# RunhuiWang/DeltaPQ

Measured on AMD Instinct MI355X. Metric: queries/sec, SIFT1M-shaped m=8 k=256 topk=100, higher is better.
Workload: dtype f64 sum of f32 table entries (u8 code decode; the reference's incremental f64 stack); 1 GPU

## Files before the change

deltapq_amd/_lib.py:

```python
import ctypes
import os

_HERE = os.path.dirname(os.path.abspath(__file__))
LIB_PATH = os.environ.get("DPQ_LIB_PATH") or os.path.join(_HERE, "csrc", "libdeltapq_amd.so")

c_i32, c_i64, c_f32 = ctypes.c_int32, ctypes.c_int64, ctypes.c_float
P = ctypes.POINTER


class OpenOpts(ctypes.Structure):
    _fields_ = [("device", c_i32), ("shard_rank", c_i32), ("shard_count", c_i32), ("chunks_per_segment", c_i32),
                ("cand_capacity", c_i32), ("num_codes", c_i32), ("bootstrap", c_i32), ("batch_decode", c_i32),
                ("global_offset", c_i64), ("global_n_codes", c_i64),
                ("stream_max_queries", c_i32), ("coarse_below", c_i32), ("plan_ratios", c_i32 * 3), ("boot_cap", c_i32),
                ("boot_target", c_i32), ("flags", c_i32), ("batch_tile_nodes", c_i64)]


class Info(ctypes.Structure):
    _fields_ = [("n_codes_total", c_i64), ("n_bytes_total", c_i64), ("node_lo", c_i64), ("node_hi", c_i64),
                ("algorithmic_bytes", c_i64), ("device_bytes", c_i64), ("n_diffs", c_i64), ("M", c_i32),
                ("K", c_i32), ("Ds", c_i32), ("n_segments", c_i32), ("chunks_per_segment", c_i32),
                ("max_depth", c_i32), ("device", c_i32), ("cand_capacity", c_i32), ("bootstrap_bytes", c_i64),
                ("bootstrap_stride", c_i32), ("batch_decode_mb", c_i32), ("strand_bytes", c_i64)]

# ... 205 lines not shown
    ("dpq_ip_tables", ctypes.c_int, [_VP, _VP, ctypes.c_int, _VP, _VP]),
    ("dpq_ip_tables_device", ctypes.c_int, [_VP, _VP, ctypes.c_int, _VP, _VP, _VP]),
    ("dpq_query_batch_ip", ctypes.c_int, [_VP, _VP, _VP, ctypes.c_int, ctypes.c_int, _VP, _VP, _VP, _VP]),
    ("dpq_query_batch_device_ip", ctypes.c_int, [_VP, _VP, _VP, ctypes.c_int, ctypes.c_int, _VP, _VP, _VP, _VP, _VP]),
    ("dpq_ip_scores", ctypes.c_int, [_VP, _VP, _VP, ctypes.c_int, ctypes.c_int, _VP]),
    ("dpq_profile_enable", ctypes.c_int, [_VP, ctypes.c_int]),
    ("dpq_profile_reset", ctypes.c_int, [_VP]),
    ("dpq_profile_read", ctypes.c_int, [_VP, P(Profile)]),
    ("dpq_debug_scan_time", ctypes.c_int, [_VP, ctypes.c_int, ctypes.c_int, ctypes.c_int, ctypes.c_int, P(ctypes.c_float)]),
    ("dpq_debug_scan_stamps", ctypes.c_int, [_VP, ctypes.c_int, ctypes.c_int, P(ctypes.c_ulonglong), ctypes.c_int, P(ctypes.c_float)]),
    ("dpq_debug_boot_stamps", ctypes.c_int, [_VP, ctypes.c_int, P(ctypes.c_double)]),
    ("dpq_debug_select_time", ctypes.c_int, [_VP, ctypes.c_int, ctypes.c_int, ctypes.c_int, ctypes.c_int, P(ctypes.c_float)]),
    ("dpq_debug_strand1_stamps", ctypes.c_int, [_VP, _VP, ctypes.c_int]),
    ("dpq_debug_range_keys", ctypes.c_int, [_VP, P(c_i64)]),
    ("dpq_debug_filter_tables", ctypes.c_int, [_VP, ctypes.c_int, _VP, c_i64]),
    ("dpq_debug_relabel", ctypes.c_int, [_VP, _VP, ctypes.c_int]),
]

_lib = None
_hip_runtime = None


def _bind_hip_runtime():
    global _hip_runtime
    if _hip_runtime is not None:
        return _hip_runtime
    import importlib.util
    candidates = []
    override = os.environ.get("DPQ_HIP_RUNTIME")
    if override:
# ... 52 lines not shown
```

deltapq_amd/api.py:

```python
import ctypes

import numpy as np

from . import _lib
from ._lib import DpqError, Info, OpenOpts, Profile, check


def _np_ptr(a):
    return ctypes.c_void_p(a.ctypes.data)


def device_count():
    return _lib.load().dpq_device_count()


def read_codewords(path):
    lib = _lib.load()
    M, K, Ds = _lib.c_i32(), _lib.c_i32(), _lib.c_i32()
    check(lib.dpq_read_codewords(path.encode(), M, K, Ds, None), "dpq_read_codewords")
    out = np.empty((M.value, K.value, Ds.value), dtype=np.float32)
    check(lib.dpq_read_codewords(path.encode(), M, K, Ds, _np_ptr(out)), "dpq_read_codewords")
    return out


# ... 392 lines not shown
    def info(self):
        i = Info()
        check(self._lib.dpq_get_info(self._h, i), "dpq_get_info")
        return i.as_dict()

    def query_batch(self, queries, top_k):
        q = np.ascontiguousarray(queries, dtype=np.float32)
        if q.ndim == 1:
            q = q[None, :]
        nq = q.shape[0]
        ids = np.empty((nq, top_k), dtype=np.int32)
        dists = np.empty((nq, top_k), dtype=np.float32)
        check(self._lib.dpq_query_batch(self._h, _np_ptr(q), nq, top_k, _np_ptr(ids), _np_ptr(dists)),
              "dpq_query_batch")
        return ids, dists

    def range_search(self, queries, radius):
        q = np.ascontiguousarray(queries, dtype=np.float32)
        if q.ndim == 1:
            q = q[None, :]
        nq = q.shape[0]
        r = np.ascontiguousarray(np.broadcast_to(np.asarray(radius, dtype=np.float32), (nq,)))
        res = ctypes.c_void_p()
        check(self._lib.dpq_range_search(self._h, _np_ptr(q), nq, _np_ptr(r), res), "dpq_range_search")
        try:
            n = _lib.c_i32()
            pl, pi, pd = ctypes.c_void_p(), ctypes.c_void_p(), ctypes.c_void_p()
            check(self._lib.dpq_range_result_get(res, n, pl, pi, pd), "dpq_range_result_get")
            lims = np.ctypeslib.as_array(ctypes.cast(pl, ctypes.POINTER(_lib.c_i64)), (n.value + 1,)).copy()
            total = int(lims[-1])
# ... 1119 lines not shown
```

deltapq_amd/csrc/dpq_capi.cpp:

```cpp
#include "dpq_capi_internal.h"

namespace {

thread_local std::string g_last_error;

}

int fail(int code, const std::string& msg) {
    g_last_error = msg;
    return code;
}

uint64_t next_index_serial() {
    static std::atomic<uint64_t> next{1};
    return next++;
}

bool dev_mode() {
    const char* dev = getenv("DPQ_DEV");
    return dev && atoi(dev) != 0;
}

namespace {

// ... 22 lines not shown
        geti("DPQ_BOOT_TARGET", &t.boot_target);
        geti("DPQ_BOOT_VARIANT", &t.boot_variant);
        if (const char* e = getenv("DPQ_BATCH_TILE_NODES")) t.batch_tile_nodes = std::max<int64_t>(1, atoll(e));
        int v = 1;
        geti("DPQ_RELABEL", &v); t.relabel = t.relabel && v != 0;
        v = 1; geti("DPQ_FUSE_QUANTISE", &v); t.fuse_quantise = t.fuse_quantise && v != 0;
        v = 1; geti("DPQ_ASYNC_OVERLAP", &v); t.async_overlap = t.async_overlap && v != 0;
        v = 0; geti("DPQ_BOOT_FULLSORT", &v); t.boot_fullsort = t.boot_fullsort || v != 0;
        v = 1; geti("DPQ_TIGHTEN", &v); t.tighten = t.tighten && v != 0;
        geti("DPQ_SELECT_THREADS", &t.select_threads);
        geti("DPQ_SELECT_FAST", &t.select_fast);
        v = 1; geti("DPQ_STRANDS", &v); t.strands = t.strands && v != 0;
        t.force_strands = t.force_strands || v == 2;
        v = 1; geti("DPQ_STRAND1", &v); t.strand1 = t.strand1 && v != 0;
        geti("DPQ_S1_DEBUG", &t.s1_debug);
    }
    return t;
}

void use_lane(dpq_index* x, int lane) {
    if (lane == x->active_lane) return;
    x->dbg_groups = x->dbg_boot_slots = 0;
    x->active_lane = lane;
}

int ensure_workspace(dpq_index* x, int slots, int cap) {
    Workspace& w = x->ws();
    if (slots <= w.slots && cap <= w.cap) return DPQ_OK;
    slots = std::max(slots, w.slots);
    cap = std::max(cap, w.cap);
    x->dbg_groups = x->dbg_boot_slots = 0;
    DevBuf<uint8_t> batch_raw = std::move(w.d_batch_raw);
    w = Workspace();
    w.d_batch_raw = std::move(batch_raw);
    int rc;
    if ((rc = w.d_lut32.alloc((size_t)slots * x->M * 256))) return rc;
    if (x->d_relabel && (rc = w.d_lut32r.alloc((size_t)slots * x->M * 256))) return rc;
    if ((rc = w.d_lut_min.alloc((size_t)slots * x->M * 4))) return rc;
    if ((rc = w.d_lut_stat.alloc((size_t)slots * x->M))) return rc;
    if ((rc = w.d_qtab.alloc((size_t)(slots / dpq::queries_per_group(x->M) + 1) *
                             (dpq::qtab_bytes_per_group(x->M) / sizeof(uint4)))))
        return rc;
    if ((rc = w.d_cand_count.alloc((size_t)slots * dpq::kRegionStride))) return rc;
    if ((rc = w.d_cand_key.alloc((size_t)slots * cap))) return rc;
    if ((rc = w.d_scratch.alloc((size_t)slots * cap))) return rc;
    if ((rc = w.d_overflow.alloc((size_t)slots))) return rc;
    if ((rc = w.d_tight.alloc((size_t)slots * dpq::kTightWords))) return rc;
    if ((rc = w.d_thr_key.alloc((size_t)slots))) return rc;
    if ((rc = w.d_dbg_thr.alloc((size_t)slots))) return rc;
    if (!x->h_overflow) DPQ_HIP(hipHostMalloc(reinterpret_cast<void**>(&x->h_overflow), sizeof(uint32_t) * 4096));
    if (!x->d_counters) {
        if ((rc = x->d_counters.alloc(2))) return rc;
        DPQ_HIP(hipMemset(x->d_counters, 0, 16));
    }
// ... 248 lines not shown
    if (stride > INT32_MAX) return fail(DPQ_ERR_NOMEM, "candidate buffer too large");
    if ((rc = ensure_workspace(x, b->nqp, (int)stride))) return rc;
    b->stride = x->ws().cap;
    if (b->scratch && (rc = ensure_batch_raw(x))) return rc;
    return DPQ_OK;
}

int build_tables(dpq_index* x, const Batch& b, const TableSource& src, hipStream_t stream, bool row_stats = true) {
    Workspace& w = x->ws();
    int rc;
    if (b.one_tile && (rc = ensure_plain_image(x, stream))) return rc;
    {
        Timer t(x, stream, 0);
        const uint8_t* relabel = b.scratch ? x->d_relabel.get() : nullptr;
        uint32_t* tight = x->tune.tighten ? w.d_tight.get() : nullptr;
        if (src.d_tables)
            DPQ_HIP(dpq::launch_tables_ingest(src.d_tables, b.nq, b.nqp, x->M, x->K, w.d_lut32, w.d_lut_min, w.d_overflow,
                                              relabel, w.d_lut32r, tight, src.d_bad, stream));
        else
            DPQ_HIP(dpq::launch_lut_build(x->d_codebook, src.d_queries, b.nq, b.nqp, x->M, x->K, x->Ds, w.d_lut32,
                                          w.d_lut_min, nullptr, w.d_overflow, relabel, w.d_lut32r, tight, stream));
        if (row_stats) DPQ_HIP(dpq::launch_row_stats(w.d_lut32, b.nq, x->M, w.d_lut_stat, stream));
    }
    if (x->prof) x->prof_acc.lut_launches++;
    return DPQ_OK;
}

dpq::ScanArgs batch_scan_args(const dpq_index* x, const Batch& b) {
    const Workspace& w = x->ws();
    dpq::ScanArgs sa{};
    sa.img = x->img;
    if (b.one_tile) sa.img.raw = x->d_plain_image;
    sa.fp32_accum = x->plain ? 1 : 0;
    sa.lut32 = b.labelled ? w.d_lut32r.get() : w.d_lut32.get();
    sa.lut_min = w.d_lut_min;
    sa.lut_stat = w.d_lut_stat;
    sa.thr_key = w.d_thr_key;
// ... 1731 lines not shown
        int rc;
        if ((rc = d_rec.alloc(records))) return rc;
        dpq::ScanArgs sa{};
        sa.img.M = x->M;
        sa.lut_min = w.d_lut_min;
        sa.lut_stat = w.d_lut_stat;
        sa.thr_key = w.d_dbg_thr;
        sa.n_queries = w.dbg_qtab_nq;
        DPQ_HIP(dpq::launch_saturation_debug(sa, slots, d_rec, nullptr));
        DPQ_HIP(hipMemcpy(static_cast<char*>(out) + tables, d_rec.get(), records, hipMemcpyDeviceToHost));
    }
    return DPQ_OK;
    });
}

int dpq_debug_relabel(dpq_index* x, unsigned char* out, int bytes) {
    return guarded([&]() -> int {
    DPQ_DEV_ONLY();
    if (!x || !out || bytes < x->M * 256) return fail(DPQ_ERR_ARG, "bad argument");
    if (!x->d_relabel) return fail(DPQ_ERR_STATE, "the handle has no label map");
    DPQ_HIP(hipSetDevice(x->device));
    DPQ_HIP(hipDeviceSynchronize());
    DPQ_HIP(hipMemcpy(out, x->d_relabel.get(), (size_t)x->M * 256, hipMemcpyDeviceToHost));
    return DPQ_OK;
    });
}

int dpq_debug_range_keys(dpq_index* x, int64_t* max_keys) {
    DPQ_DEV_ONLY();
    if (!x || !max_keys) return fail(DPQ_ERR_ARG, "NULL argument");
// ... 102 lines not shown
```

deltapq_amd/csrc/dpq_capi_internal.h:

```cpp
#pragma once
#include <hip/hip_runtime.h>

#include <algorithm>
#include <atomic>
#include <chrono>
#include <cmath>
#include <cstdio>
#include <cstdlib>
#include <cstring>
#include <iterator>
#include <memory>
#include <new>
#include <numeric>
#include <stdexcept>
#include <string>
#include <type_traits>
#include <vector>

#include "../../include/deltapq_amd.h"
#include "dpq_build.h"
#include "dpq_filter.h"
#include "dpq_flat.h"
#include "dpq_format.h"
#include "dpq_kernels.h"
// ... 145 lines not shown
uint64_t next_index_serial();

struct Tuning {
    int stream_max = 4;
    int coarse_below = 128;
    int plan_ratios[3] = {0, 0, 0};
    int boot_cap = 0, boot_target = 0;
    int boot_variant = 1;
    int select_threads = 0;
    int select_fast = 1;
    int64_t batch_tile_nodes = (int64_t)16 << 20;
    bool relabel = true, fuse_quantise = true, async_overlap = true, boot_fullsort = false, tighten = true, strands = true,
         force_strands = false;
    bool strand1 = true;
    int s1_debug = 0;
};

struct RangeWs {
    DevBuf<int32_t> slot_query;
    DevBuf<uint64_t> thr_key;
    DevBuf<int64_t> out_off;
    DevBuf<uint32_t> max_count;
    DevBuf<int64_t> lims;
    DevBuf<uint32_t> cand_count;
    DevBuf<uint64_t> cand_key;
    DevBuf<int32_t> out_ids;
    DevBuf<float> out_dists;
    DevBuf<uint64_t> scratch;
    size_t key_n = 0, out_n = 0, scratch_n = 0;
    int64_t last_max_keys = 0;
// ... 10 lines not shown
};

struct TableSource {
    const float* d_queries = nullptr;
    const float* d_tables = nullptr;
    uint32_t* d_bad = nullptr;
    const float* h_tables = nullptr;
};

struct Workspace {
    int slots = 0, cap = 0;
    DevBuf<float> d_lut32;
    DevBuf<float> d_lut32r;
    DevBuf<float> d_lut_min;
    DevBuf<float> d_lut_stat;
    DevBuf<uint4> d_qtab;
    DevBuf<uint32_t> d_cand_count;
    DevBuf<uint32_t> d_overflow;
    DevBuf<uint32_t> d_tight;
    DevBuf<uint64_t> d_cand_key, d_thr_key;
    DevBuf<uint64_t> d_scratch;
    DevBuf<uint8_t> d_batch_raw;
    int dbg_qtab_groups = 0, dbg_qtab_levels = 0;
    int dbg_qtab_nq = 0;
    DevBuf<uint64_t> d_dbg_thr;
};

struct dpq_index {
    Tuning tune;
    const uint64_t serial = next_index_serial();
// ... 144 lines not shown
```

deltapq_amd/csrc/dpq_kernels.h:

```cpp
#pragma once
#include <hip/hip_runtime.h>

#include <cstdint>

#include "dpq_format.h"

namespace dpq {

constexpr int kScanThreads = 1024;
constexpr int kScanWaves = kScanThreads / 64;
constexpr int kMaxTopK = 2048;
constexpr int kSelectThreads = 512;
constexpr int kMaxSplits = 256;
constexpr int kRegionStride = 1 + kMaxSplits;
constexpr int kLevel0Nodes = 3840;
constexpr int kSortMax = 4096;
constexpr int queries_per_group(int M) { return M <= 8 ? 64 : 32; }
constexpr int kTightBuckets = 8;
constexpr int kTightSplits = 32;
constexpr int kTightWords = kTightSplits * kTightBuckets / 4;
constexpr int kS1Replicas = 8, kS1ReplicaWords = 512;
constexpr int kS1HistWords = kS1Replicas * kS1ReplicaWords;
static_assert(queries_per_group(8) * kTightWords >= kS1HistWords, "strand1's histogram exceeds what one query group clears");
constexpr int kLutQueries = 8;
constexpr int kLutMinParts = 4;

struct DeviceImage {
    const uint8_t* nib = nullptr;
    const uint8_t* par = nullptr;
    const uint8_t* carry = nullptr;
    const uint8_t* mask = nullptr;
    const uint8_t* delta = nullptr;
    const uint64_t* seg_delta_off = nullptr;
    const uint8_t* seg_ckpt = nullptr;
    const uint8_t* raw = nullptr;
    const uint64_t* st_ckpt = nullptr;
    const uint32_t* st_mask = nullptr;
    const uint16_t* st_depth = nullptr;
    const uint32_t* st_pbase = nullptr;
    const uint8_t* st_delta = nullptr;
// ... 106 lines not shown
    const int64_t* out_off;
    const uint32_t* cand_count;
    const uint64_t* cand_key;
    int64_t cand_stride;
    int32_t region_off, region_cap, n_regions;
    int32_t lds_keys;
    int32_t* out_ids;
    float* out_dists;
    int64_t out_n;
    uint64_t* scratch;
    int64_t n_codes_total;
};

hipError_t launch_lut_build(const float* d_codebook, const float* d_queries, int nq, int n_slots, int M, int K, int Ds,
                            float* d_lut32, float* d_lut_min, uint32_t* d_cand_count, uint32_t* d_overflow,
                            const uint8_t* d_relabel, float* d_lut_labels, uint32_t* d_tight_hist,
                            hipStream_t stream);
hipError_t launch_decode_list(const DeviceImage& img, const uint32_t* seg_list, int n_seg, const uint8_t* relabel,
                              uint32_t* out_code, hipStream_t stream);
hipError_t launch_decode_segments(const DeviceImage& img, const uint32_t* seg_list, int n_seg, uint32_t* out_id,
                                  uint32_t* out_code, hipStream_t stream);
hipError_t launch_stream(const ScanArgs& a, int n_slots, hipStream_t stream);
hipError_t launch_strand(const ScanArgs& a, int n_slots, hipStream_t stream);
int stream_queries_per_pass(int M, int n_slots);
hipError_t launch_strand1(const ScanArgs& a, int n_slots, hipStream_t stream);
int strand1_workgroups(int n_strips);
constexpr int kStrand1Regions = 256;
hipError_t launch_quantise(const ScanArgs& a, int n_slot_groups, hipStream_t stream);
hipError_t launch_row_stats(const float* d_lut32, int nq, int M, float* d_lut_stat, hipStream_t stream);
hipError_t launch_scan(const ScanArgs& a, int n_slot_groups, int splits, hipStream_t stream);
size_t qtab_bytes_per_group(int M);
hipError_t launch_saturation_debug(const ScanArgs& a, int n_slots, unsigned char* d_out, hipStream_t stream);
// ... 14 lines not shown
```

deltapq_amd/csrc/dpq_kernels.hip:

```cpp
#include "dpq_kernels.h"
#include "dpq_wave_decoder.h"

#include <atomic>
#include <type_traits>
#include <cfloat>
#include <cmath>

namespace dpq {

static hipError_t ensure_dynamic_lds(const void* fn, size_t bytes, std::atomic<bool>* done);


__device__ __forceinline__ uint32_t and_or(uint32_t a, uint32_t mask, uint32_t c) {
    uint32_t r;
    asm("v_and_or_b32 %0, %1, %2, %3" : "=v"(r) : "v"(a), "s"(mask), "v"(c));
    return r;
}

__device__ __forceinline__ uint64_t make_key(float d, uint32_t id) {
    return ((uint64_t)__float_as_uint(d) << 32) | (uint64_t)id;
}

__device__ __forceinline__ float lut_min_of(const float* __restrict__ lut_min, size_t q, int M, int m) {
    const float4 p = *reinterpret_cast<const float4*>(lut_min + (q * M + m) * kLutMinParts);
    return fminf(fminf(p.x, p.y), fminf(p.z, p.w));
}

__global__ __launch_bounds__(256) void lut_build_kernel(const float* __restrict__ codebook,
                                                         const float* __restrict__ queries, int nq, int n_slots, int M,
                                                         int K, int Ds, float* __restrict__ lut,
                                                         float* __restrict__ lut_min, uint32_t* __restrict__ cand_count,
                                                         uint32_t* __restrict__ overflow, const uint8_t* __restrict__ relabel,
                                                         float* __restrict__ lut_labels, uint32_t* __restrict__ tight_hist) {
#ifndef DPQ_UNDER_SCAN_PRIO
#define DPQ_UNDER_SCAN_PRIO 3
#endif
    __builtin_amdgcn_s_setprio(DPQ_UNDER_SCAN_PRIO);
    const int q0 = blockIdx.x * kLutQueries, m = blockIdx.y, k = threadIdx.x;
    if (m == 0 && k < kLutQueries && q0 + k < n_slots) {
        if (cand_count) cand_count[q0 + k] = 0;
        if (overflow) overflow[q0 + k] = 0;
    }
    if (m == 0 && tight_hist)
        for (int i = k; i < kLutQueries * kTightWords; i += 256)
            if (q0 * kTightWords + i < n_slots * kTightWords) tight_hist[(size_t)q0 * kTightWords + i] = 0;
    if (q0 >= nq) return;
    float acc[kLutQueries];
#pragma unroll
    for (int j = 0; j < kLutQueries; ++j) acc[j] = 0.0f;
    if (k < K) {
        const float* c = codebook + ((size_t)m * K + k) * Ds;
        const float* qv = queries + (size_t)q0 * M * Ds + (size_t)m * Ds;
        const size_t qstride = (size_t)M * Ds;
        auto step = [&](float& a, float cv, float qd) {
            const float diff = __fsub_rn(cv, qd);
            const double sq = __dmul_rn((double)diff, (double)diff);
            a = (float)__dadd_rn((double)a, sq);
        };
        if ((Ds & 3) == 0) {
            const float4* c4 = reinterpret_cast<const float4*>(c);
            for (int d = 0; d < Ds; d += 4) {
                const float4 v = c4[d >> 2];
#pragma unroll
                for (int j = 0; j < kLutQueries; ++j) {
                    const float* qj = qv + (size_t)min(j, nq - 1 - q0) * qstride + d;
                    step(acc[j], v.x, qj[0]);
                    step(acc[j], v.y, qj[1]);
                    step(acc[j], v.z, qj[2]);
                    step(acc[j], v.w, qj[3]);
                }
            }
        } else {
            for (int d = 0; d < Ds; ++d) {
                const float cv = c[d];
#pragma unroll
                for (int j = 0; j < kLutQueries; ++j) step(acc[j], cv, qv[(size_t)min(j, nq - 1 - q0) * qstride + d]);
            }
        }
    } else {
#pragma unroll
        for (int j = 0; j < kLutQueries; ++j) acc[j] = INFINITY;
    }
#pragma unroll
    for (int j = 0; j < kLutQueries; ++j) {
        if (q0 + j < nq) lut[((size_t)(q0 + j) * M + m) * 256 + k] = acc[j];
        if (lut_labels && q0 + j < nq) lut_labels[((size_t)(q0 + j) * M + m) * 256 + relabel[m * 256 + k]] = acc[j];
        uint32_t v = __float_as_uint(acc[j]);
#pragma unroll
        for (int o = 32; o > 0; o >>= 1) v = min(v, (uint32_t)__shfl_xor((int)v, o));
        if ((k & 63) == 0 && q0 + j < nq) lut_min[((size_t)(q0 + j) * M + m) * kLutMinParts + (k >> 6)] = __uint_as_float(v);
    }
}

template <int M>
__global__ __launch_bounds__(64) void decode_segments_kernel(const DeviceImage img,
                                                              const uint32_t* __restrict__ seg_list,
                                                              uint32_t* __restrict__ out_id,
                                                              uint32_t* __restrict__ out_code) {
    constexpr int W = Cfg<M>::W;
    const int lane = threadIdx.x;
    const uint32_t seg = seg_list ? seg_list[blockIdx.x] : blockIdx.x;
    const int cps = img.chunks_per_segment;
    WaveDecoder<M> dec;
    if (!img.raw) dec.begin_segment(img, seg, lane);
    for (int c = 0; c < cps; ++c) {
        const int64_t node = ((int64_t)seg * cps + c) * 64 + lane;
// ... 93 lines not shown
    const float mn = fs.s32 != 0.0f ? min_m : 0.0f;
    const double od = (double)mn * (double)fs.s32;
    float of = (float)od;
    if ((double)of < od) of = __uint_as_float(__float_as_uint(of) + 1u);
    const double sd = (m == 0 ? (double)fs.bias : 0.0) - 0.5 - (double)of;
    float sf = (float)sd;
    if ((double)sf > sd) sf = __uint_as_float(__float_as_uint(sf) + (sf > 0.0f ? -1 : 1));
    return sf;
}

template <int M>
__device__ __forceinline__ uint32_t filter_field(float tv, float sc, float of, uint32_t clamp) {
    const float fv = fminf(__fmaf_rn(tv, sc, of), (float)clamp);
    return __builtin_amdgcn_cvt_pk_u8_f32(fv, 0u, 0u);
}

constexpr int kSatRank = 32;

template <int M>
__global__ __launch_bounds__(64 * M) void row_stat_kernel(const float* __restrict__ lut32, float* __restrict__ lut_stat) {
    const int q = blockIdx.x, m = threadIdx.x >> 6, lane = threadIdx.x & 63;
    const float* row = lut32 + ((size_t)q * M + m) * 256;
    uint32_t x[4];
#pragma unroll
    for (int j = 0; j < 4; ++j) x[j] = __float_as_uint(row[lane + 64 * j]) & 0x7fffffffu;
    uint32_t r = 0;
    for (int b = 30; b >= 0; --b) {
        const uint32_t c = r | (1u << b);
        int n = 0;
#pragma unroll
        for (int j = 0; j < 4; ++j) n += __popcll(__ballot(x[j] >= c));
        if (n >= kSatRank) r = c;
// ... 2636 lines not shown
}

size_t scan_lds_bytes(int M) { return M <= 8 ? ScanLds<8>::kBytes : ScanLds<16>::kBytes; }

size_t select_lds_bytes(int M, int top_k, int n_shared) {
    size_t kp = 1;
    while (kp < (size_t)top_k) kp <<= 1;
    const size_t n_keys = n_shared > 0 ? (size_t)std::min(n_shared, kSortMax) : (size_t)select_list_keys(top_k);
    const size_t area = n_shared > 0 ? kp : (size_t)select_area_keys(top_k);
    const size_t select_bytes = area * 8 + 266 * 4, table_bytes = n_shared > 0 ? (size_t)M * 256 * 4 : 0;
    return n_keys * 8 + std::max(select_bytes, table_bytes) + 16;
}

hipError_t launch_lut_build(const float* d_codebook, const float* d_queries, int nq, int n_slots, int M, int K, int Ds,
                            float* d_lut32, float* d_lut_min, uint32_t* d_cand_count, uint32_t* d_overflow,
                            const uint8_t* d_relabel, float* d_lut_labels, uint32_t* d_tight_hist, hipStream_t stream) {
    if (nq <= 0) return hipSuccess;
    n_slots = std::max(n_slots, nq);
    hipLaunchKernelGGL(lut_build_kernel, dim3((unsigned)((n_slots + kLutQueries - 1) / kLutQueries), (unsigned)M),
                       dim3(256), 0, stream, d_codebook, d_queries, nq, n_slots, M, K, Ds, d_lut32, d_lut_min,
                       d_cand_count, d_overflow, d_relabel, d_relabel ? d_lut_labels : nullptr, d_tight_hist);
    return hipGetLastError();
}

hipError_t launch_decode_segments(const DeviceImage& img, const uint32_t* seg_list, int n_seg, uint32_t* out_id,
                                  uint32_t* out_code, hipStream_t stream) {
    if (n_seg <= 0) return hipSuccess;
    if (img.M == 8)
        hipLaunchKernelGGL(decode_segments_kernel<8>, dim3((unsigned)n_seg), dim3(64), 0, stream, img, seg_list,
                           out_id, out_code);
    else if (img.M == 16)
        hipLaunchKernelGGL(decode_segments_kernel<16>, dim3((unsigned)n_seg), dim3(64), 0, stream, img, seg_list,
                           out_id, out_code);
    else
        return hipErrorInvalidValue;
    return hipGetLastError();
// ... 228 lines not shown
```

deltapq_amd/csrc/dpq_tables.h:

```cpp
#pragma once
#include <hip/hip_runtime.h>

#include <cstdint>

namespace dpq {

constexpr int kIpQueries = 4;

hipError_t launch_tables_ingest(const float* d_tables, int nq, int n_slots, int M, int K, float* d_lut32, float* d_lut_min,
                                uint32_t* d_overflow, const uint8_t* d_relabel, float* d_lut_labels, uint32_t* d_tight_hist,
                                uint32_t* d_bad, hipStream_t stream);

hipError_t launch_ip_tables(const float* d_codebook, const float* d_queries, int nq, int M, int K, int Ds, float* d_tables,
                            float* d_bias, hipStream_t stream);

hipError_t launch_ip_scores(const float* d_bias, const float* d_gaps, const int32_t* d_ids, int nq, int top_k,
                            float* d_scores, hipStream_t stream);

}
```

deltapq_amd/csrc/dpq_tables.hip:

```cpp
#include "dpq_tables.h"

#include <algorithm>
#include <cmath>

#include "dpq_kernels.h"

namespace dpq {

#ifndef DPQ_UNDER_SCAN_PRIO
#define DPQ_UNDER_SCAN_PRIO 3
#endif

__global__ __launch_bounds__(256) void tables_ingest_kernel(const float* __restrict__ tables, int nq, int n_slots, int M,
                                                             int K, float* __restrict__ lut, float* __restrict__ lut_min,
                                                             uint32_t* __restrict__ overflow,
                                                             const uint8_t* __restrict__ relabel,
                                                             float* __restrict__ lut_labels,
                                                             uint32_t* __restrict__ tight_hist, uint32_t* __restrict__ bad) {
    __builtin_amdgcn_s_setprio(DPQ_UNDER_SCAN_PRIO);
    const int q = blockIdx.x, m = blockIdx.y, k = threadIdx.x;
    if (m == 0) {
        if (k == 0 && overflow) overflow[q] = 0;
        if (tight_hist)
            for (int i = k; i < kTightWords; i += 256) tight_hist[(size_t)q * kTightWords + i] = 0;
    }
    if (q >= nq) return;
    float v = INFINITY;
    if (k < K) {
        v = tables[((size_t)q * M + m) * K + k];
        if (!(v >= 0.0f)) {
            v = INFINITY;
            *bad = 1u;
        }
    }
    uint32_t b = __float_as_uint(v);
    if (b == 0x80000000u) b = 0u;
    v = __uint_as_float(b);
    lut[((size_t)q * M + m) * 256 + k] = v;
    if (lut_labels) lut_labels[((size_t)q * M + m) * 256 + relabel[m * 256 + k]] = v;
#pragma unroll
    for (int o = 32; o > 0; o >>= 1) b = min(b, (uint32_t)__shfl_xor((int)b, o));
    if ((k & 63) == 0) lut_min[((size_t)q * M + m) * kLutMinParts + (k >> 6)] = __uint_as_float(b);
}

__global__ __launch_bounds__(256) void ip_tables_kernel(const float* __restrict__ codebook, const float* __restrict__ queries,
                                                         int nq, int M, int K, int Ds, float* __restrict__ tables,
                                                         float* __restrict__ bias) {
    __shared__ float wave_top[4][kIpQueries];
    const int q0 = blockIdx.x * kIpQueries, k = threadIdx.x;
    const int nj = min(kIpQueries, nq - q0);
    const size_t qstride = (size_t)M * Ds;
    double B[kIpQueries];
#pragma unroll
    for (int j = 0; j < kIpQueries; ++j) B[j] = 0.0;
    for (int m = 0; m < M; ++m) {
        double acc[kIpQueries];
#pragma unroll
// ... 31 lines not shown
        for (int j = 0; j < kIpQueries; ++j)
            if (j < nj) bias[q0 + j] = (float)B[j];
    }
}

__global__ __launch_bounds__(256) void ip_scores_kernel(const float* __restrict__ bias, const float* __restrict__ gaps,
                                                         const int32_t* __restrict__ ids, int top_k, int64_t n,
                                                         float* __restrict__ scores) {
    const int64_t i = (int64_t)blockIdx.x * 256 + threadIdx.x;
    if (i >= n) return;
    scores[i] = ids[i] < 0 ? -INFINITY : (float)__dsub_rn((double)bias[i / top_k], (double)gaps[i]);
}

hipError_t launch_tables_ingest(const float* d_tables, int nq, int n_slots, int M, int K, float* d_lut32, float* d_lut_min,
                                uint32_t* d_overflow, const uint8_t* d_relabel, float* d_lut_labels, uint32_t* d_tight_hist,
                                uint32_t* d_bad, hipStream_t stream) {
    if (nq <= 0) return hipSuccess;
    n_slots = std::max(n_slots, nq);
    hipLaunchKernelGGL(tables_ingest_kernel, dim3((unsigned)n_slots, (unsigned)M), dim3(256), 0, stream, d_tables, nq, n_slots,
                       M, K, d_lut32, d_lut_min, d_overflow, d_relabel, d_relabel ? d_lut_labels : nullptr, d_tight_hist,
                       d_bad);
    return hipGetLastError();
}

hipError_t launch_ip_tables(const float* d_codebook, const float* d_queries, int nq, int M, int K, int Ds, float* d_tables,
                            float* d_bias, hipStream_t stream) {
    if (nq <= 0) return hipSuccess;
    hipLaunchKernelGGL(ip_tables_kernel, dim3((unsigned)((nq + kIpQueries - 1) / kIpQueries)), dim3(256), 0, stream,
                       d_codebook, d_queries, nq, M, K, Ds, d_tables, d_bias);
    return hipGetLastError();
}

hipError_t launch_ip_scores(const float* d_bias, const float* d_gaps, const int32_t* d_ids, int nq, int top_k,
                            float* d_scores, hipStream_t stream) {
    const int64_t n = (int64_t)nq * top_k;
    if (n <= 0) return hipSuccess;
// ... 7 lines not shown
```

include/deltapq_amd.h:

```cpp
#ifndef DELTAPQ_AMD_H
#define DELTAPQ_AMD_H

#include <stdint.h>

#ifdef __cplusplus
extern "C" {
#endif

#define DPQ_VERSION 100

typedef enum dpq_status {
    DPQ_OK = 0,
    DPQ_ERR_ARG = -1,
    DPQ_ERR_IO = -2,
    DPQ_ERR_FORMAT = -3,
    DPQ_ERR_NO_DEVICE = -4,
    DPQ_ERR_HIP = -5,
    DPQ_ERR_NOMEM = -6,
    DPQ_ERR_STATE = -7,
    DPQ_ERR_TOPK = -8
} dpq_status;

typedef struct dpq_index dpq_index;
typedef struct dpq_soa dpq_soa;
// ... 376 lines not shown
int dpq_query_batch_device_ip(dpq_index* idx, const dpq_filter* filter, const float* d_queries, int nq, int top_k,
                              int32_t* d_ids, float* d_scores, float* d_gaps, float* d_bias, void* hip_stream);
int dpq_ip_scores(const float* bias, const float* gaps, const int32_t* ids, int nq, int top_k, float* scores_out);

int dpq_profile_enable(dpq_index* idx, int on);
int dpq_profile_reset(dpq_index* idx);
int dpq_profile_read(dpq_index* idx, dpq_profile* out);

int dpq_debug_scan_time(dpq_index* idx, int nq, int pass_all, int reps, int splits, float* ms_out);
int dpq_debug_scan_stamps(dpq_index* idx, int nq, int splits, unsigned long long* out, int n_out, float* ms_out);
int dpq_debug_boot_stamps(dpq_index* idx, int nq, double* out);
int dpq_debug_select_time(dpq_index* idx, int nq, int top_k, int flags, int reps, float* ms_out);
int dpq_debug_range_keys(dpq_index* idx, int64_t* max_keys);
int dpq_debug_strand1_stamps(dpq_index* idx, unsigned long long* out, int n_words);
int dpq_debug_filter_tables(dpq_index* idx, int lane, void* out, int64_t bytes);
int dpq_debug_relabel(dpq_index* idx, unsigned char* out, int bytes);

#ifdef __cplusplus
}
#endif
#endif
```

Before: 6.894 million queries/s.

## Fuse row stats into LUT build and restructure it to one wave per two queries

The LUT build kernel now has each 64-lane wave own two queries and all 256 codewords (four per lane), instead of each of 256 threads owning one codeword for eight queries. The per-row min, a saturation-rank statistic and a nearest-code index are computed in a shared DPP-based epilogue, so the separate row_stats kernel launch is removed. The tables-ingest kernel is reshaped the same way. The aim is to drop one kernel launch and one pass over the LUT, and to reuse codebook loads across queries. In exchange, lut_min now stores the full-row minimum in all four slots rather than per-quarter minima, and an extra nearest-code buffer is written on every batch.

```diff
diff --git a/deltapq_amd/_lib.py b/deltapq_amd/_lib.py
--- a/deltapq_amd/_lib.py
+++ b/deltapq_amd/_lib.py
@@ -243,6 +243,7 @@
     ("dpq_debug_strand1_stamps", ctypes.c_int, [_VP, _VP, ctypes.c_int]),
     ("dpq_debug_range_keys", ctypes.c_int, [_VP, P(c_i64)]),
     ("dpq_debug_filter_tables", ctypes.c_int, [_VP, ctypes.c_int, _VP, c_i64]),
+    ("dpq_debug_batch_tables", ctypes.c_int, [_VP, ctypes.c_int, ctypes.c_int, _VP, _VP, _VP, _VP]),
     ("dpq_debug_relabel", ctypes.c_int, [_VP, _VP, ctypes.c_int]),
 ]
 
diff --git a/deltapq_amd/api.py b/deltapq_amd/api.py
--- a/deltapq_amd/api.py
+++ b/deltapq_amd/api.py
@@ -430,6 +430,16 @@
         check(self._lib.dpq_query_batch(self._h, _np_ptr(q), nq, top_k, _np_ptr(ids), _np_ptr(dists)),
               "dpq_query_batch")
         return ids, dists
+
+    def debug_batch_tables(self, nq, lane=0):
+        M = self.info()["M"]
+        lut32 = np.empty((nq, M, 256), dtype=np.float32)
+        lut_min = np.empty((nq, M, 4), dtype=np.float32)
+        lut_stat = np.empty((nq, M), dtype=np.float32)
+        lut_near = np.empty((nq, M), dtype=np.uint32)
+        check(self._lib.dpq_debug_batch_tables(self._h, lane, nq, _np_ptr(lut32), _np_ptr(lut_min), _np_ptr(lut_stat),
+                                               _np_ptr(lut_near)), "dpq_debug_batch_tables")
+        return lut32, lut_min, lut_stat, lut_near
 
     def range_search(self, queries, radius):
         q = np.ascontiguousarray(queries, dtype=np.float32)
diff --git a/deltapq_amd/csrc/dpq_capi.cpp b/deltapq_amd/csrc/dpq_capi.cpp
--- a/deltapq_amd/csrc/dpq_capi.cpp
+++ b/deltapq_amd/csrc/dpq_capi.cpp
@@ -60,6 +60,7 @@
         t.force_strands = t.force_strands || v == 2;
         v = 1; geti("DPQ_STRAND1", &v); t.strand1 = t.strand1 && v != 0;
         geti("DPQ_S1_DEBUG", &t.s1_debug);
+        geti("DPQ_LUT_WAVE_QUERIES", &t.lut_wave_queries);
     }
     return t;
 }
@@ -84,6 +85,7 @@
     if (x->d_relabel && (rc = w.d_lut32r.alloc((size_t)slots * x->M * 256))) return rc;
     if ((rc = w.d_lut_min.alloc((size_t)slots * x->M * 4))) return rc;
     if ((rc = w.d_lut_stat.alloc((size_t)slots * x->M))) return rc;
+    if ((rc = w.d_lut_near.alloc((size_t)slots * x->M))) return rc;
     if ((rc = w.d_qtab.alloc((size_t)(slots / dpq::queries_per_group(x->M) + 1) *
                              (dpq::qtab_bytes_per_group(x->M) / sizeof(uint4)))))
         return rc;
@@ -362,13 +364,15 @@
         Timer t(x, stream, 0);
         const uint8_t* relabel = b.scratch ? x->d_relabel.get() : nullptr;
         uint32_t* tight = x->tune.tighten ? w.d_tight.get() : nullptr;
+        float* stat = row_stats ? w.d_lut_stat.get() : nullptr;
+        uint32_t* near = w.d_lut_near.get();
         if (src.d_tables)
             DPQ_HIP(dpq::launch_tables_ingest(src.d_tables, b.nq, b.nqp, x->M, x->K, w.d_lut32, w.d_lut_min, w.d_overflow,
-                                              relabel, w.d_lut32r, tight, src.d_bad, stream));
+                                              relabel, w.d_lut32r, tight, src.d_bad, stat, near, stream));
         else
             DPQ_HIP(dpq::launch_lut_build(x->d_codebook, src.d_queries, b.nq, b.nqp, x->M, x->K, x->Ds, w.d_lut32,
-                                          w.d_lut_min, nullptr, w.d_overflow, relabel, w.d_lut32r, tight, stream));
-        if (row_stats) DPQ_HIP(dpq::launch_row_stats(w.d_lut32, b.nq, x->M, w.d_lut_stat, stream));
+                                          w.d_lut_min, nullptr, w.d_overflow, relabel, w.d_lut32r, tight, stat, near,
+                                          x->tune.lut_wave_queries, stream));
     }
     if (x->prof) x->prof_acc.lut_launches++;
     return DPQ_OK;
@@ -2130,6 +2134,23 @@
     });
 }
 
+int dpq_debug_batch_tables(dpq_index* x, int lane, int nq, float* lut32, float* lut_min, float* lut_stat, uint32_t* lut_near) {
+    return guarded([&]() -> int {
+    DPQ_DEV_ONLY();
+    if (!x || lane < 0 || lane > 1 || nq <= 0) return fail(DPQ_ERR_ARG, "bad argument");
+    const Workspace& w = x->lane[lane];
+    if (!w.d_lut32 || nq > w.slots) return fail(DPQ_ERR_STATE, "the lane has answered no batch of that many queries");
+    DPQ_HIP(hipSetDevice(x->device));
+    DPQ_HIP(hipDeviceSynchronize());
+    const size_t rows = (size_t)nq * x->M;
+    if (lut32) DPQ_HIP(hipMemcpy(lut32, w.d_lut32.get(), rows * 256 * sizeof(float), hipMemcpyDeviceToHost));
+    if (lut_min) DPQ_HIP(hipMemcpy(lut_min, w.d_lut_min.get(), rows * dpq::kLutMinParts * sizeof(float), hipMemcpyDeviceToHost));
+    if (lut_stat) DPQ_HIP(hipMemcpy(lut_stat, w.d_lut_stat.get(), rows * sizeof(float), hipMemcpyDeviceToHost));
+    if (lut_near) DPQ_HIP(hipMemcpy(lut_near, w.d_lut_near.get(), rows * sizeof(uint32_t), hipMemcpyDeviceToHost));
+    return DPQ_OK;
+    });
+}
+
 int dpq_debug_relabel(dpq_index* x, unsigned char* out, int bytes) {
     return guarded([&]() -> int {
     DPQ_DEV_ONLY();
diff --git a/deltapq_amd/csrc/dpq_capi_internal.h b/deltapq_amd/csrc/dpq_capi_internal.h
--- a/deltapq_amd/csrc/dpq_capi_internal.h
+++ b/deltapq_amd/csrc/dpq_capi_internal.h
@@ -183,6 +183,7 @@
          force_strands = false;
     bool strand1 = true;
     int s1_debug = 0;
+    int lut_wave_queries = 0;
 };
 
 struct RangeWs {
@@ -223,6 +224,7 @@
     DevBuf<float> d_lut32r;
     DevBuf<float> d_lut_min;
     DevBuf<float> d_lut_stat;
+    DevBuf<uint32_t> d_lut_near;
     DevBuf<uint4> d_qtab;
     DevBuf<uint32_t> d_cand_count;
     DevBuf<uint32_t> d_overflow;
diff --git a/deltapq_amd/csrc/dpq_kernels.h b/deltapq_amd/csrc/dpq_kernels.h
--- a/deltapq_amd/csrc/dpq_kernels.h
+++ b/deltapq_amd/csrc/dpq_kernels.h
@@ -24,6 +24,8 @@
 static_assert(queries_per_group(8) * kTightWords >= kS1HistWords, "strand1's histogram exceeds what one query group clears");
 constexpr int kLutQueries = 8;
 constexpr int kLutMinParts = 4;
+constexpr int kSatRank = 32;
+constexpr int kLutWaveQueries = 2;
 
 struct DeviceImage {
     const uint8_t* nib = nullptr;
@@ -160,8 +162,8 @@
 
 hipError_t launch_lut_build(const float* d_codebook, const float* d_queries, int nq, int n_slots, int M, int K, int Ds,
                             float* d_lut32, float* d_lut_min, uint32_t* d_cand_count, uint32_t* d_overflow,
-                            const uint8_t* d_relabel, float* d_lut_labels, uint32_t* d_tight_hist,
-                            hipStream_t stream);
+                            const uint8_t* d_relabel, float* d_lut_labels, uint32_t* d_tight_hist, float* d_lut_stat,
+                            uint32_t* d_lut_near, int wave_queries, hipStream_t stream);
 hipError_t launch_decode_list(const DeviceImage& img, const uint32_t* seg_list, int n_seg, const uint8_t* relabel,
                               uint32_t* out_code, hipStream_t stream);
 hipError_t launch_decode_segments(const DeviceImage& img, const uint32_t* seg_list, int n_seg, uint32_t* out_id,
diff --git a/deltapq_amd/csrc/dpq_kernels.hip b/deltapq_amd/csrc/dpq_kernels.hip
--- a/deltapq_amd/csrc/dpq_kernels.hip
+++ b/deltapq_amd/csrc/dpq_kernels.hip
@@ -1,4 +1,5 @@
 #include "dpq_kernels.h"
+#include "dpq_row_epilogue.h"
 #include "dpq_wave_decoder.h"
 
 #include <atomic>
@@ -26,30 +27,37 @@
     return fminf(fminf(p.x, p.y), fminf(p.z, p.w));
 }
 
-__global__ __launch_bounds__(256) void lut_build_kernel(const float* __restrict__ codebook,
-                                                         const float* __restrict__ queries, int nq, int n_slots, int M,
-                                                         int K, int Ds, float* __restrict__ lut,
-                                                         float* __restrict__ lut_min, uint32_t* __restrict__ cand_count,
-                                                         uint32_t* __restrict__ overflow, const uint8_t* __restrict__ relabel,
-                                                         float* __restrict__ lut_labels, uint32_t* __restrict__ tight_hist) {
+template <int QW>
+__global__ __launch_bounds__(64 * (kLutQueries / QW)) void lut_build_kernel(
+    const float* __restrict__ codebook, const float* __restrict__ queries, int nq, int n_slots, int M, int K, int Ds,
+    float* __restrict__ lut, float* __restrict__ lut_min, uint32_t* __restrict__ cand_count, uint32_t* __restrict__ overflow,
+    const uint8_t* __restrict__ relabel, float* __restrict__ lut_labels, uint32_t* __restrict__ tight_hist,
+    float* __restrict__ lut_stat, uint32_t* __restrict__ lut_near) {
 #ifndef DPQ_UNDER_SCAN_PRIO
 #define DPQ_UNDER_SCAN_PRIO 3
 #endif
     __builtin_amdgcn_s_setprio(DPQ_UNDER_SCAN_PRIO);
-    const int q0 = blockIdx.x * kLutQueries, m = blockIdx.y, k = threadIdx.x;
-    if (m == 0 && k < kLutQueries && q0 + k < n_slots) {
-        if (cand_count) cand_count[q0 + k] = 0;
-        if (overflow) overflow[q0 + k] = 0;
+    constexpr int THREADS = 64 * (kLutQueries / QW);
+    const int qb = blockIdx.x * kLutQueries, m = blockIdx.y, t = threadIdx.x, lane = t & 63;
+    if (m == 0 && t < kLutQueries && qb + t < n_slots) {
+        if (cand_count) cand_count[qb + t] = 0;
+        if (overflow) overflow[qb + t] = 0;
     }
     if (m == 0 && tight_hist)
-        for (int i = k; i < kLutQueries * kTightWords; i += 256)
-            if (q0 * kTightWords + i < n_slots * kTightWords) tight_hist[(size_t)q0 * kTightWords + i] = 0;
+        for (int i = t; i < kLutQueries * kTightWords; i += THREADS)
+            if (qb * kTightWords + i < n_slots * kTightWords) tight_hist[(size_t)qb * kTightWords + i] = 0;
+    const int q0 = qb + __builtin_amdgcn_readfirstlane(t >> 6) * QW;
     if (q0 >= nq) return;
-    float acc[kLutQueries];
-#pragma unroll
-    for (int j = 0; j < kLutQueries; ++j) acc[j] = 0.0f;
-    if (k < K) {
-        const float* c = codebook + ((size_t)m * K + k) * Ds;
+    const int rows = min(QW, nq - q0);
+    float acc[QW][4];
+#pragma unroll
+    for (int i = 0; i < QW; ++i)
+#pragma unroll
+        for (int j = 0; j < 4; ++j) acc[i][j] = 0.0f;
+    {
+        const float* c[4];
+#pragma unroll
+        for (int j = 0; j < 4; ++j) c[j] = codebook + ((size_t)m * K + min(lane + 64 * j, K - 1)) * Ds;
         const float* qv = queries + (size_t)q0 * M * Ds + (size_t)m * Ds;
         const size_t qstride = (size_t)M * Ds;
         auto step = [&](float& a, float cv, float qd) {
@@ -58,38 +66,50 @@
             a = (float)__dadd_rn((double)a, sq);
         };
         if ((Ds & 3) == 0) {
-            const float4* c4 = reinterpret_cast<const float4*>(c);
             for (int d = 0; d < Ds; d += 4) {
-                const float4 v = c4[d >> 2];
-#pragma unroll
-                for (int j = 0; j < kLutQueries; ++j) {
-                    const float* qj = qv + (size_t)min(j, nq - 1 - q0) * qstride + d;
-                    step(acc[j], v.x, qj[0]);
-                    step(acc[j], v.y, qj[1]);
-                    step(acc[j], v.z, qj[2]);
-                    step(acc[j], v.w, qj[3]);
+                float4 v[4];
+#pragma unroll
+                for (int j = 0; j < 4; ++j) v[j] = reinterpret_cast<const float4*>(c[j])[d >> 2];
+#pragma unroll
+                for (int i = 0; i < QW; ++i) {
+                    const float* qi = qv + (size_t)min(i, rows - 1) * qstride + d;
+                    const float q0v = qi[0], q1v = qi[1], q2v = qi[2], q3v = qi[3];
+#pragma unroll
+                    for (int j = 0; j < 4; ++j) {
+                        step(acc[i][j], v[j].x, q0v);
+                        step(acc[i][j], v[j].y, q1v);
+                        step(acc[i][j], v[j].z, q2v);
+                        step(acc[i][j], v[j].w, q3v);
+                    }
                 }
             }
         } else {
             for (int d = 0; d < Ds; ++d) {
-                const float cv = c[d];
-#pragma unroll
-                for (int j = 0; j < kLutQueries; ++j) step(acc[j], cv, qv[(size_t)min(j, nq - 1 - q0) * qstride + d]);
-            }
-        }
-    } else {
-#pragma unroll
-        for (int j = 0; j < kLutQueries; ++j) acc[j] = INFINITY;
-    }
-#pragma unroll
-    for (int j = 0; j < kLutQueries; ++j) {
-        if (q0 + j < nq) lut[((size_t)(q0 + j) * M + m) * 256 + k] = acc[j];
-        if (lut_labels && q0 + j < nq) lut_labels[((size_t)(q0 + j) * M + m) * 256 + relabel[m * 256 + k]] = acc[j];
-        uint32_t v = __float_as_uint(acc[j]);
-#pragma unroll
-        for (int o = 32; o > 0; o >>= 1) v = min(v, (uint32_t)__shfl_xor((int)v, o));
-        if ((k & 63) == 0 && q0 + j < nq) lut_min[((size_t)(q0 + j) * M + m) * kLutMinParts + (k >> 6)] = __uint_as_float(v);
-    }
+                float cv[4];
+#pragma unroll
+                for (int j = 0; j < 4; ++j) cv[j] = c[j][d];
+#pragma unroll
+                for (int i = 0; i < QW; ++i) {
+                    const float qd = qv[(size_t)min(i, rows - 1) * qstride + d];
+#pragma unroll
+                    for (int j = 0; j < 4; ++j) step(acc[i][j], cv[j], qd);
+                }
+            }
+        }
+    }
+#pragma unroll
+    for (int j = 0; j < 4; ++j) {
+        const int k = lane + 64 * j;
+#pragma unroll
+        for (int i = 0; i < QW; ++i) {
+            if (k >= K) acc[i][j] = INFINITY;
+            if (i < rows) {
+                lut[((size_t)(q0 + i) * M + m) * 256 + k] = acc[i][j];
+                if (lut_labels) lut_labels[((size_t)(q0 + i) * M + m) * 256 + relabel[m * 256 + k]] = acc[i][j];
+            }
+        }
+    }
+    row_epilogue<QW>(acc, lane, rows, (size_t)q0 * M + m, (size_t)M, lut_min, lut_stat, lut_near);
 }
 
 template <int M>
@@ -213,8 +233,6 @@
     const float fv = fminf(__fmaf_rn(tv, sc, of), (float)clamp);
     return __builtin_amdgcn_cvt_pk_u8_f32(fv, 0u, 0u);
 }
-
-constexpr int kSatRank = 32;
 
 template <int M>
 __global__ __launch_bounds__(64 * M) void row_stat_kernel(const float* __restrict__ lut32, float* __restrict__ lut_stat) {
@@ -2881,12 +2899,21 @@
 
 hipError_t launch_lut_build(const float* d_codebook, const float* d_queries, int nq, int n_slots, int M, int K, int Ds,
                             float* d_lut32, float* d_lut_min, uint32_t* d_cand_count, uint32_t* d_overflow,
-                            const uint8_t* d_relabel, float* d_lut_labels, uint32_t* d_tight_hist, hipStream_t stream) {
+                            const uint8_t* d_relabel, float* d_lut_labels, uint32_t* d_tight_hist, float* d_lut_stat,
+                            uint32_t* d_lut_near, int wave_queries, hipStream_t stream) {
     if (nq <= 0) return hipSuccess;
+    if (K < 1 || K > 256) return hipErrorInvalidValue;
     n_slots = std::max(n_slots, nq);
-    hipLaunchKernelGGL(lut_build_kernel, dim3((unsigned)((n_slots + kLutQueries - 1) / kLutQueries), (unsigned)M),
-                       dim3(256), 0, stream, d_codebook, d_queries, nq, n_slots, M, K, Ds, d_lut32, d_lut_min,
-                       d_cand_count, d_overflow, d_relabel, d_relabel ? d_lut_labels : nullptr, d_tight_hist);
+    if (M != 8) d_lut_stat = nullptr;
+    const dim3 grid((unsigned)((n_slots + kLutQueries - 1) / kLutQueries), (unsigned)M);
+    if ((wave_queries > 0 ? wave_queries : kLutWaveQueries) == 2)
+        hipLaunchKernelGGL(lut_build_kernel<2>, grid, dim3(256), 0, stream, d_codebook, d_queries, nq, n_slots, M, K, Ds,
+                           d_lut32, d_lut_min, d_cand_count, d_overflow, d_relabel, d_relabel ? d_lut_labels : nullptr,
+                           d_tight_hist, d_lut_stat, d_lut_near);
+    else
+        hipLaunchKernelGGL(lut_build_kernel<8>, grid, dim3(64), 0, stream, d_codebook, d_queries, nq, n_slots, M, K, Ds,
+                           d_lut32, d_lut_min, d_cand_count, d_overflow, d_relabel, d_relabel ? d_lut_labels : nullptr,
+                           d_tight_hist, d_lut_stat, d_lut_near);
     return hipGetLastError();
 }
 
diff --git a/deltapq_amd/csrc/dpq_row_epilogue.h b/deltapq_amd/csrc/dpq_row_epilogue.h
--- /dev/null
+++ b/deltapq_amd/csrc/dpq_row_epilogue.h
@@ -0,0 +1,63 @@
+#pragma once
+#include <hip/hip_runtime.h>
+
+#include <cstdint>
+
+#include "dpq_kernels.h"
+
+namespace dpq {
+
+__device__ __forceinline__ uint32_t wave_min_u32(uint32_t v) {
+    v = min(v, (uint32_t)__builtin_amdgcn_update_dpp(0, (int)v, 0xB1, 0xf, 0xf, true));
+    v = min(v, (uint32_t)__builtin_amdgcn_update_dpp(0, (int)v, 0x4E, 0xf, 0xf, true));
+    v = min(v, (uint32_t)__builtin_amdgcn_update_dpp(0, (int)v, 0x141, 0xf, 0xf, true));
+    v = min(v, (uint32_t)__builtin_amdgcn_update_dpp(0, (int)v, 0x140, 0xf, 0xf, true));
+    const uint32_t a = (uint32_t)__builtin_amdgcn_readlane((int)v, 0), b = (uint32_t)__builtin_amdgcn_readlane((int)v, 16);
+    const uint32_t c = (uint32_t)__builtin_amdgcn_readlane((int)v, 32), d = (uint32_t)__builtin_amdgcn_readlane((int)v, 48);
+    return min(min(a, b), min(c, d));
+}
+
+template <int R>
+__device__ __forceinline__ void row_epilogue(const float (&e)[R][4], int lane, int rows, size_t row0, size_t row_step,
+                                             float* __restrict__ lut_min, float* __restrict__ lut_stat,
+                                             uint32_t* __restrict__ lut_near) {
+    uint32_t x[R][4];
+#pragma unroll
+    for (int i = 0; i < R; ++i) {
+        uint32_t mn = 0xffffffffu, nr = 0xffffffffu;
+#pragma unroll
+        for (int j = 0; j < 4; ++j) {
+            const uint32_t b = __float_as_uint(e[i][j]);
+            x[i][j] = b & 0x7fffffffu;
+            mn = min(mn, b);
+            nr = min(nr, (b & 0xffffff00u) | (uint32_t)(lane + 64 * j));
+        }
+        mn = wave_min_u32(mn);
+        if (lut_near) nr = wave_min_u32(nr);
+        if (lane == 0 && i < rows) {
+            const float f = __uint_as_float(mn);
+            static_assert(kLutMinParts == 4, "one 16-byte store");
+            reinterpret_cast<float4*>(lut_min)[row0 + i * row_step] = make_float4(f, f, f, f);
+            if (lut_near) lut_near[row0 + i * row_step] = nr & 0xffu;
+        }
+    }
+    if (!lut_stat) return;
+    uint32_t r[R];
+#pragma unroll
+    for (int i = 0; i < R; ++i) r[i] = 0;
+    for (int b = 30; b >= 0; --b) {
+#pragma unroll
+        for (int i = 0; i < R; ++i) {
+            const uint32_t c = r[i] | (1u << b);
+            int n = 0;
+#pragma unroll
+            for (int j = 0; j < 4; ++j) n += __popcll(__ballot(x[i][j] >= c));
+            if (n >= kSatRank) r[i] = c;
+        }
+    }
+#pragma unroll
+    for (int i = 0; i < R; ++i)
+        if (lane == 0 && i < rows) lut_stat[row0 + i * row_step] = __uint_as_float(r[i]);
+}
+
+}
diff --git a/deltapq_amd/csrc/dpq_tables.h b/deltapq_amd/csrc/dpq_tables.h
--- a/deltapq_amd/csrc/dpq_tables.h
+++ b/deltapq_amd/csrc/dpq_tables.h
@@ -9,7 +9,7 @@
 
 hipError_t launch_tables_ingest(const float* d_tables, int nq, int n_slots, int M, int K, float* d_lut32, float* d_lut_min,
                                 uint32_t* d_overflow, const uint8_t* d_relabel, float* d_lut_labels, uint32_t* d_tight_hist,
-                                uint32_t* d_bad, hipStream_t stream);
+                                uint32_t* d_bad, float* d_lut_stat, uint32_t* d_lut_near, hipStream_t stream);
 
 hipError_t launch_ip_tables(const float* d_codebook, const float* d_queries, int nq, int M, int K, int Ds, float* d_tables,
                             float* d_bias, hipStream_t stream);
diff --git a/deltapq_amd/csrc/dpq_tables.hip b/deltapq_amd/csrc/dpq_tables.hip
--- a/deltapq_amd/csrc/dpq_tables.hip
+++ b/deltapq_amd/csrc/dpq_tables.hip
@@ -4,6 +4,7 @@
 #include <cmath>
 
 #include "dpq_kernels.h"
+#include "dpq_row_epilogue.h"
 
 namespace dpq {
 
@@ -16,31 +17,37 @@
                                                              uint32_t* __restrict__ overflow,
                                                              const uint8_t* __restrict__ relabel,
                                                              float* __restrict__ lut_labels,
-                                                             uint32_t* __restrict__ tight_hist, uint32_t* __restrict__ bad) {
+                                                             uint32_t* __restrict__ tight_hist, uint32_t* __restrict__ bad,
+                                                             float* __restrict__ lut_stat, uint32_t* __restrict__ lut_near) {
     __builtin_amdgcn_s_setprio(DPQ_UNDER_SCAN_PRIO);
-    const int q = blockIdx.x, m = blockIdx.y, k = threadIdx.x;
-    if (m == 0) {
-        if (k == 0 && overflow) overflow[q] = 0;
+    const int q = blockIdx.x, t = threadIdx.x, lane = t & 63;
+    const int m = blockIdx.y * 4 + __builtin_amdgcn_readfirstlane(t >> 6);
+    if (blockIdx.y == 0) {
+        if (t == 0 && overflow) overflow[q] = 0;
         if (tight_hist)
-            for (int i = k; i < kTightWords; i += 256) tight_hist[(size_t)q * kTightWords + i] = 0;
+            for (int i = t; i < kTightWords; i += 256) tight_hist[(size_t)q * kTightWords + i] = 0;
     }
-    if (q >= nq) return;
-    float v = INFINITY;
-    if (k < K) {
-        v = tables[((size_t)q * M + m) * K + k];
-        if (!(v >= 0.0f)) {
-            v = INFINITY;
-            *bad = 1u;
+    if (q >= nq || m >= M) return;
+    float e[1][4];
+#pragma unroll
+    for (int j = 0; j < 4; ++j) {
+        const int k = lane + 64 * j;
+        float v = INFINITY;
+        if (k < K) {
+            v = tables[((size_t)q * M + m) * K + k];
+            if (!(v >= 0.0f)) {
+                v = INFINITY;
+                *bad = 1u;
+            }
         }
+        uint32_t b = __float_as_uint(v);
+        if (b == 0x80000000u) b = 0u;
+        v = __uint_as_float(b);
+        lut[((size_t)q * M + m) * 256 + k] = v;
+        if (lut_labels) lut_labels[((size_t)q * M + m) * 256 + relabel[m * 256 + k]] = v;
+        e[0][j] = v;
     }
-    uint32_t b = __float_as_uint(v);
-    if (b == 0x80000000u) b = 0u;
-    v = __uint_as_float(b);
-    lut[((size_t)q * M + m) * 256 + k] = v;
-    if (lut_labels) lut_labels[((size_t)q * M + m) * 256 + relabel[m * 256 + k]] = v;
-#pragma unroll
-    for (int o = 32; o > 0; o >>= 1) b = min(b, (uint32_t)__shfl_xor((int)b, o));
-    if ((k & 63) == 0) lut_min[((size_t)q * M + m) * kLutMinParts + (k >> 6)] = __uint_as_float(b);
+    row_epilogue<1>(e, lane, 1, (size_t)q * M + m, (size_t)M, lut_min, lut_stat, lut_near);
 }
 
 __global__ __launch_bounds__(256) void ip_tables_kernel(const float* __restrict__ codebook, const float* __restrict__ queries,
@@ -102,12 +109,13 @@
 
 hipError_t launch_tables_ingest(const float* d_tables, int nq, int n_slots, int M, int K, float* d_lut32, float* d_lut_min,
                                 uint32_t* d_overflow, const uint8_t* d_relabel, float* d_lut_labels, uint32_t* d_tight_hist,
-                                uint32_t* d_bad, hipStream_t stream) {
+                                uint32_t* d_bad, float* d_lut_stat, uint32_t* d_lut_near, hipStream_t stream) {
     if (nq <= 0) return hipSuccess;
     n_slots = std::max(n_slots, nq);
-    hipLaunchKernelGGL(tables_ingest_kernel, dim3((unsigned)n_slots, (unsigned)M), dim3(256), 0, stream, d_tables, nq, n_slots,
-                       M, K, d_lut32, d_lut_min, d_overflow, d_relabel, d_relabel ? d_lut_labels : nullptr, d_tight_hist,
-                       d_bad);
+    if (M != 8) d_lut_stat = nullptr;
+    hipLaunchKernelGGL(tables_ingest_kernel, dim3((unsigned)n_slots, (unsigned)((M + 3) / 4)), dim3(256), 0, stream, d_tables,
+                       nq, n_slots, M, K, d_lut32, d_lut_min, d_overflow, d_relabel, d_relabel ? d_lut_labels : nullptr,
+                       d_tight_hist, d_bad, d_lut_stat, d_lut_near);
     return hipGetLastError();
 }
 
diff --git a/include/deltapq_amd.h b/include/deltapq_amd.h
--- a/include/deltapq_amd.h
+++ b/include/deltapq_amd.h
@@ -414,6 +414,8 @@
 int dpq_debug_range_keys(dpq_index* idx, int64_t* max_keys);
 int dpq_debug_strand1_stamps(dpq_index* idx, unsigned long long* out, int n_words);
 int dpq_debug_filter_tables(dpq_index* idx, int lane, void* out, int64_t bytes);
+int dpq_debug_batch_tables(dpq_index* idx, int lane, int nq, float* lut32, float* lut_min, float* lut_stat,
+                           uint32_t* lut_near);
 int dpq_debug_relabel(dpq_index* idx, unsigned char* out, int bytes);
 
 #ifdef __cplusplus
```

Measured after the change: 6.823 million queries/s. 0.99x the previous value.
